# mklarqvist/StormBitmaps

Measured on AMD Instinct MI355X. Metric: 64-bit bitmap words/s, XX^T upper-tri pairwise AND+popcount (10000x65536), higher is better.
Workload: dtype u64 (bits as exact FP4 0/1 MFMA operands, f32 accumulate < 2^24); 1 GPU; STORM_contiguous_t N=10000 M=65536 dense draws=32768 seed=42 (BASELINE configs[1], README `benchmark 65536 10000`); entry_point=storm_hip_pairw_dense_launch == STORM_contig_pairw_intersect_cardinality_blocked, kernel_variant=4, work_items=14520

## Files before the change

### stormbitmaps_amd/csrc/storm_hip_mfma.hip

```cpp
#include "storm_hip_internal.h"

#include <algorithm>
#include <chrono>
#include <cstring>
#include <exception>
#include <type_traits>
#include <utility>

namespace storm {

#ifdef STORM_HIP_PROBES
__device__ unsigned long long g_clock_probe[4];
#define STORM_CLOCK_BEGIN()                                  \
    const uint64_t ck_t0 = __builtin_amdgcn_s_memtime();     \
    const uint64_t ck_r0 = __builtin_amdgcn_s_memrealtime()
#define STORM_CLOCK_END()                                                                           \
    do {                                                                                            \
        if (threadIdx.x == 0) {                                                                     \
            atomicAdd(&g_clock_probe[0], (unsigned long long)(__builtin_amdgcn_s_memtime() - ck_t0)); \
            atomicAdd(&g_clock_probe[1], (unsigned long long)(__builtin_amdgcn_s_memrealtime() - ck_r0)); \
            atomicAdd(&g_clock_probe[2], 1ull);                                                     \
        }                                                                                           \
    } while (0)
#else
#define STORM_CLOCK_BEGIN() do {} while (0)
#define STORM_CLOCK_END() do {} while (0)
#endif

static hipError_t wait_stream(storm_hip_ctx_t* ctx) {
    if (ctx->sync_poll_us > 0) {
        const auto t0 = std::chrono::steady_clock::now();
        for (uint32_t spin = 0;; ++spin) {
            const hipError_t q = hipStreamQuery(ctx->stream);
            if (q != hipErrorNotReady) return q;
            if ((spin & 15u) == 15u &&
                std::chrono::duration<double, std::micro>(std::chrono::steady_clock::now() - t0).count() > ctx->sync_poll_us)
                break;
        }
    }
    return hipStreamSynchronize(ctx->stream);
}

constexpr int kMfmaThreads = 512;
constexpr int kTileStageBytes = kTile * kStageBytes;
constexpr int kRing = 4;

typedef int v8i __attribute__((ext_vector_type(8)));
typedef int v4i __attribute__((ext_vector_type(4)));
typedef float v16f __attribute__((ext_vector_type(16)));

using gptr_t = const __attribute__((address_space(1))) void*;
using lptr_t = __attribute__((address_space(3))) void*;

#include "tile_window.inc"

__device__ __forceinline__ uint32_t spread8_fp4(uint32_t b, uint32_t nib = 2u) {
    uint32_t x = (b | (b << 12)) & 0x000F000Fu;
    x = (x | (x << 6)) & 0x03030303u;
    x = (x | (x << 3)) & 0x11111111u;
    return x * nib;
}

struct ExpandOwn {
    uint32_t rank, count, unit_shift, modulo_units;
};
constexpr ExpandOwn kExpandAll = {0u, 1u, 7u, 0u};

__global__ __launch_bounds__(256) void expand_fp4_kernel(const uint64_t* __restrict__ X,
                                                         uint64_t stride_words,
                                                         uint64_t n_rows_src, uint64_t n_rows_dst,
                                                         uint4* __restrict__ X4, ExpandOwn own,
                                                         uint32_t nib = 2u, uint64_t out_pitch_u4 = 0,
                                                         uint64_t h_begin = 0, uint64_t h_end = 0,
                                                         uint64_t h_dst0 = 0) {
    if (out_pitch_u4 == 0) out_pitch_u4 = stride_words * 2;
    const uint64_t halves_per_row = stride_words * 2;
    if (h_end == 0) h_end = halves_per_row;
    const uint32_t shift = own.unit_shift;
    const uint64_t units = (h_end - h_begin + (1ull << shift) - 1) >> shift;
// ... 379 lines not shown
        STORM_LGKM(0);
    }
#undef STORM_FETCH16
#undef STORM_MUL16
#undef STORM_LGKM
#undef STORM_LGKM_STR

    uint64_t mine = 0;
#pragma unroll
    for (int m = 0; m < 4; ++m) {
        uint32_t part = 0;
#pragma unroll
        for (int n = 0; n < 4; ++n)
#pragma unroll
            for (int r = 0; r < 4; ++r) part += (uint32_t)acc[m][n][r];
        mine += part;
    }
#pragma unroll
    for (int o = 32; o > 0; o >>= 1) mine += __shfl_down(mine, o, 64);
    if (lane == 0 && mine != 0)
        atomicAdd(&slots[(item_idx * (uint32_t)kStripWaves + wave) & (kSlots - 1)],
                  (unsigned long long)mine);
}

constexpr int kSb16ImgRing = 3;
constexpr int kSb16BitRing = 3;
[[maybe_unused]] constexpr int kSb16BitStage = kStripBRows * 64;
constexpr uint32_t kSb16ImgBytes = kSb16ImgRing * kStripStageBytes;
constexpr uint32_t kSb16Mask = 0x22222222u;

__device__ __forceinline__ v4i sb16_inflate(v4i w, uint32_t rot) {
    v4i e;
    e.x = (int)(__builtin_amdgcn_alignbit((uint32_t)w.x, (uint32_t)w.x, rot) & kSb16Mask);
    e.y = (int)(__builtin_amdgcn_alignbit((uint32_t)w.y, (uint32_t)w.y, rot) & kSb16Mask);
    e.z = (int)(__builtin_amdgcn_alignbit((uint32_t)w.z, (uint32_t)w.z, rot) & kSb16Mask);
    e.w = (int)(__builtin_amdgcn_alignbit((uint32_t)w.w, (uint32_t)w.w, rot) & kSb16Mask);
    return e;
}

#define STORM_SB16_WAVES 4
#define STORM_SB16_NAME strip16_bits_kernel
#include "strip16_bits_kernel.inc"
#undef STORM_SB16_WAVES
#undef STORM_SB16_NAME
#define STORM_SB16_WAVES 8
#define STORM_SB16_NAME strip16_bits2_kernel
#include "strip16_bits_kernel.inc"
#undef STORM_SB16_WAVES
#undef STORM_SB16_NAME

constexpr uint32_t kSr16SliceBytes = 16;
constexpr uint32_t kSr16PerTile = kStripRowsATile / kStripBRows;
constexpr uint32_t kSr16StageBytes = kStripBRows * 64;
constexpr uint32_t kSr16ImgBytes = 3 * kSr16StageBytes;
constexpr uint32_t kSr16BitRing = 3;
constexpr uint32_t kSr16BitStage = 4 * 256;

__device__ __forceinline__ v4i sr16_inflate(uint32_t w) {
    v4i e;
    e.x = (int)(__builtin_amdgcn_alignbit(w, w, 31u) & kSb16Mask);
    e.y = (int)(w & kSb16Mask);
    e.z = (int)(__builtin_amdgcn_alignbit(w, w, 1u) & kSb16Mask);
    e.w = (int)(__builtin_amdgcn_alignbit(w, w, 2u) & kSb16Mask);
    return e;
}
#include "strip16_rows_kernel.inc"

[[maybe_unused]] constexpr int kT16Ring = 4;
constexpr int kT16RowBytes = 128;
[[maybe_unused]] constexpr int kT16StageBytes = kTile * kT16RowBytes;

#ifdef STORM_HIP_PROBES
#include "../../tools/probes/tile16_fp4.hip"
#endif

[[maybe_unused]] constexpr int kTbThreads = 256;
constexpr int kTbRing = 4;
constexpr int kTbRowBytes = 64;
constexpr int kTbImageBytes = kTile * kTbRowBytes;
constexpr int kTbStageBytes = 2 * kTbImageBytes;

template <int C>
__device__ __forceinline__ v4i tb_inflate(v4i w) {
    typedef unsigned v4u __attribute__((ext_vector_type(4)));
    if constexpr (C == 3) return (v4i)(((v4u)w >> 1u) & 0x44444444u);
    else return w & (int)(0x11111111u << C);
}
template <int C>
__device__ __forceinline__ int tb_scale() {
    return C == 0 ? 128 : C == 1 ? 127 : 126;
}

template <int MB>
__device__ __forceinline__ void tb_store_interior(const v16f (&acc)[MB][4], uint8_t* lds_wave,
                                                  uint32_t* __restrict__ out_tile, uint64_t ld,
                                                  uint32_t lane, const uint32_t* __restrict__ row_counts,
                                                  uint32_t i0, uint32_t j0, uint32_t and_weight) {
    uint32_t* w32 = reinterpret_cast<uint32_t*>(lds_wave);
    const uint4* r128 = reinterpret_cast<const uint4*>(lds_wave);
    uint32_t nj[4] = {0u, 0u, 0u, 0u};
    if (row_counts) {
#pragma unroll
        for (int n = 0; n < 4; ++n) nj[n] = row_counts[j0 + (uint32_t)n * 32u + (lane & 31u)];
    }
#pragma unroll
    for (int m = 0; m < MB; ++m) {
#pragma unroll
// ... 1586 lines not shown
            l.n = (uint32_t)items.size();
            if (l.n) {
                if (int rc_up = upload_bytes(ctx, l.d, items.data(), items.size() * sizeof(StripItem))) return rc_up;
                STORM_HIP_TRY(hipStreamSynchronize(ctx->stream));
            }
            l.key = rq;
        }
        STORM_HIP_TRY(hipStreamWaitEvent(ctx->stream, l.landed, 0));
        if (l.n) {
            hipLaunchKernelGGL(strip16_bits_kernel, dim3(l.n), dim3(kStripThreads), (size_t)ctx->k2_lds_pad, ctx->stream,
                               reinterpret_cast<const uint8_t*>(m->d), pitch, l.d.d, ctx->d_slots,
                               (unsigned long long*)nullptr, (uint32_t)kSlots);
            STORM_HIP_TRY(hipGetLastError());
        }
        n_total += l.n;
    }
    ctx->last_info[0] = n_total;
    ctx->last_info[1] = ctx->k2_stages_per_item;
    ctx->last_info[2] = 1;
    ctx->last_info[3] = n_panels;
    return launch_fold_slots(ctx, d_total);
}

int strip_operands_of(const storm_hip_ctx_t* ctx) {
    if (ctx->k2_strip_operands == 6) return 5;
    if (ctx->k2_strip_operands != 0) return ctx->k2_strip_operands;
    return (ctx->k2_ring == kStripRingDefault && ctx->k2_shape == 16) ? 5 : 4;
}
int launch_pairw_mfma(storm_hip_ctx_t* ctx, const storm_hip_matrix_s* m, uint32_t shard_rank,
                      uint32_t shard_count, uint64_t* d_total) {
    const int strip_mode = ctx->variant == 5 ? 2 : ctx->variant == 4 ? 1 : 0;
    const int operands = strip_operands_of(ctx);
    if (strip_mode == 1 && (operands == 1 || operands == 2 || operands == 3 || operands == 5) && !ctx->k2_persistent && ctx->k2_debug == 0 &&
        (m->n_rows + kStripATile - 1) / kStripATile * kStripATile <= m->n_rows_pad &&
        m->stride_words * 8 * (uint64_t)kStripBRows < (1ull << 32))
    {
        const bool wide = operands == 5 && ctx->k2_strip_operands == 6 && (m->n_rows + 511u) / 512u * 512u <= m->n_rows_pad;
        ctx->k2_operands_used = wide ? 6 : operands;
        return launch_pairw_bits(ctx, m, shard_rank, shard_count, wide ? 6 : operands, d_total);
    }
    ctx->k2_operands_used = 4;
    const uint64_t tile = strip_mode == 2 ? 512 : kStripATile;
    const uint64_t n_rows4 = (m->n_rows + tile - 1) / tile * tile;
    std::vector<RowRange> ranges;
    if (m->n_rows > 1) ranges.push_back({0, m->n_rows});
    return launch_pairw_mfma_ranges(ctx, m->d, m->stride_words, m->n_rows_pad, n_rows4, ranges,
                                    shard_rank, shard_count, strip_mode, d_total, m->generation,
                                    m->n_words);
}

}

#ifdef STORM_HIP_PROBES
extern "C" int storm_hip_probe_clock(uint64_t out[3]) {
    unsigned long long v[4] = {0, 0, 0, 0};
    if (hipDeviceSynchronize() != hipSuccess) return STORM_HIP_EINVAL;
    if (hipMemcpyFromSymbol(v, HIP_SYMBOL(storm::g_clock_probe), sizeof(v)) != hipSuccess) return STORM_HIP_EINVAL;
    out[0] = v[0];
    out[1] = v[1];
    out[2] = v[2];
    const unsigned long long z[4] = {0, 0, 0, 0};
    if (hipMemcpyToSymbol(HIP_SYMBOL(storm::g_clock_probe), z, sizeof(z)) != hipSuccess) return STORM_HIP_EINVAL;
    return STORM_HIP_OK;
}
#endif
```

### stormbitmaps_amd/csrc/strip16_rows_kernel.inc

```
__global__ __launch_bounds__(256, 4) void strip16_rows_kernel(
    const uint8_t* __restrict__ X, uint64_t row_bytes, const StripItem* __restrict__ items,
    unsigned long long* __restrict__ slots, unsigned long long* __restrict__ out, uint32_t fold_slots) {
    __shared__ __attribute__((aligned(1024))) uint8_t lds_raw[kSr16ImgBytes + kSr16BitRing * kSr16BitStage];

    constexpr uint32_t kW = 4u;
    STORM_CLOCK_BEGIN();
    const uint32_t tid = threadIdx.x;
    const uint32_t lane = tid & 63u;
    const uint32_t wave = __builtin_amdgcn_readfirstlane(tid >> 6);
    const StripItem it = items[blockIdx.x];
    const uint64_t kbyte = (uint64_t)it.ks * (uint64_t)kSr16SliceBytes;
    const uint32_t D = it.diag ? kSr16PerTile : 0u;
    const uint32_t T = D + (it.j1 - it.j0);
    const uint32_t cslot = (3u - D % 3u) % 3u;

    const uint32_t lds_base =
        (uint32_t)(uintptr_t)(__attribute__((address_space(3))) uint8_t*)&lds_raw[0];
    const uint32_t pr = wave * 16u + (lane >> 2);
    const uint32_t goff0 = pr * (uint32_t)row_bytes + (lane & 3u) * 4u;
    const uint32_t bits_rd = lds_base + kSr16ImgBytes + wave * 256u + lane * 4u;
    const uint32_t img_wr = lds_base + pr * 64u + (((lane & 3u) ^ ((0x78u >> (2u * ((pr >> 2) & 3u))) & 3u)) * 16u);

    auto issue = [&](uint32_t s, uint32_t slot) {
        const uint32_t sc = min(s, T - 1u);
        const uint32_t blk = sc < D ? it.a_row0 / (uint32_t)kStripBRows + sc : it.j1 - 1u - (sc - D);
        const uint8_t* base = X + (uint64_t)(blk * (uint32_t)kStripBRows) * row_bytes + kbyte;
        const __amdgpu_buffer_rsrc_t rsrc =
            __builtin_amdgcn_make_buffer_rsrc(const_cast<uint8_t*>(base), 0, -1, 0x00020000);
        __builtin_amdgcn_raw_ptr_buffer_load_lds(
            rsrc, (lptr_t)(lds_raw + kSr16ImgBytes + slot * kSr16BitStage + wave * 256u), 4,
            (int)goff0, 0, 0, 0);
    };

    v4i a[8];
    {
        const uint8_t* ap = X + (uint64_t)(it.a_row0 + wave * 64u + (lane & 15u)) * row_bytes + kbyte +
                            (lane >> 4) * 4u;
        uint32_t aw[8];
#pragma unroll
        for (int m = 0; m < 8; ++m)
            aw[m] = *reinterpret_cast<const uint32_t*>(ap + (uint64_t)((m & 3) * 16 + (m >> 2) * 256) * row_bytes);
        issue(0u, cslot);
        issue(1u, (cslot + 1u) % 3u);
        issue(2u, (cslot + 2u) % 3u);
#pragma unroll
        for (int m = 0; m < 8; ++m) a[m] = sr16_inflate(aw[m]);
    }

    v4f acc[8][2];
#pragma unroll
    for (int m = 0; m < 8; ++m)
#pragma unroll
        for (int n = 0; n < 2; ++n) acc[m][n] = v4f{};

    const uint32_t boff = lds_base + (lane & 15u) * 64u + (((lane >> 4) ^ ((0x78u >> (2u * ((lane & 15u) >> 2))) & 3u)) * 16u);

#pragma unroll
    for (int m = 0; m < 8; ++m) asm volatile("" ::"v"(a[m]));

#define STORM_FETCH16(dst, img, j)                                                        \
    asm volatile("ds_read_b128 %0, %1 offset:%2"                                          \
                 : "=&v"(dst)                                                             \
                 : "v"(boff), "n"((img) + (j) * 16 * 64))
#define STORM_FETCH16V(dst, img, j)                                                       \
    asm volatile("ds_read_b128 %0, %1 offset:%2"                                          \
                 : "=&v"(dst)                                                             \
                 : "v"(boff + (img)), "n"((j) * 16 * 64))
#define STORM_MUL1(m, j, frag)                                                            \
    acc[m][(j) & 1] = __builtin_amdgcn_mfma_scale_f32_16x16x128_f8f6f4(                   \
        v8i{a[m].x, a[m].y, a[m].z, a[m].w, 0, 0, 0, 0},                                  \
        v8i{frag.x, frag.y, frag.z, frag.w, 0, 0, 0, 0}, acc[m][(j) & 1], 4, 4, 0, 0, 0, 0)
#define STORM_MUL16(j, frag)                                                              \
    _Pragma("unroll") for (int m = 0; m < 8; ++m) STORM_MUL1(m, j, frag)
#define STORM_LGKM_STR(n) asm volatile("s_waitcnt lgkmcnt(" #n ")" ::: "memory")
#define STORM_LGKM(n)    \
    STORM_LGKM_STR(n);   \
    __builtin_amdgcn_sched_barrier(0)
#define STORM_VM2()                                         \
    asm volatile("s_waitcnt vmcnt(2)" ::: "memory");        \
    __builtin_amdgcn_sched_barrier(0)

    uint32_t wb = 0;
    auto build_image = [&](uint32_t s) {
        uint32_t slot = (s + cslot) % 3u;
        asm volatile("" : "+s"(slot));
        asm volatile("ds_read_b32 %0, %1" : "=&v"(wb) : "v"(bits_rd + slot * kSr16BitStage));
        STORM_LGKM(0);
        const v4i e = sr16_inflate(wb);
        asm volatile("ds_write_b128 %0, %1" ::"v"(img_wr + slot * kSr16StageBytes), "v"(e) : "memory");
        __builtin_amdgcn_sched_barrier(0);
    };

    asm volatile("s_waitcnt lgkmcnt(0)" ::: "memory");
    STORM_VM2();
    build_image(0u);
    STORM_LGKM(0);
    issue(3u, cslot);
    STORM_VM2();
    build_image(1u);

    v4i b0 = {}, b1 = {}, b2 = {};
    uint32_t t = 0;
    if (D != 0u) {
#define STORM_SR16_MASK(m, n)                                                             \
    _Pragma("unroll") for (int r = 0; r < 4; ++r) acc[m][n][r] = r < tri ? acc[m][n][r] : 0.0f;
#define STORM_SR16_WHOLE(base, j)                                                         \
    _Pragma("unroll") for (int i = 0; i < 4; ++i) {                                       \
        STORM_MUL1((base) + i, j, b0);                                                    \
        STORM_MUL1((base) + i, (j) + 1, b1);                                              \
    }
#define STORM_SR16_OWN01(base)                                                            \
    STORM_MUL1((base) + 0, 0, b0);                                                        \
    STORM_SR16_MASK((base) + 0, 0)                                                        \
    STORM_MUL1((base) + 0, 1, b1);                                                        \
    STORM_MUL1((base) + 1, 1, b1);                                                        \
    STORM_SR16_MASK((base) + 1, 1)
#define STORM_SR16_OWN23(base)                                                            \
    STORM_MUL1((base) + 0, 2, b0);                                                        \
    STORM_MUL1((base) + 1, 2, b0);                                                        \
    STORM_MUL1((base) + 2, 2, b0);                                                        \
    STORM_SR16_MASK((base) + 2, 0)                                                        \
    STORM_MUL1((base) + 0, 3, b1);                                                        \
    STORM_MUL1((base) + 1, 3, b1);                                                        \
    STORM_MUL1((base) + 2, 3, b1);                                                        \
    STORM_MUL1((base) + 3, 3, b1);                                                        \
    STORM_SR16_MASK((base) + 3, 1)
#define STORM_SR16_HEAD()                                                                 \
    STORM_LGKM(0);                                                  \
    __builtin_amdgcn_s_barrier();     \
    issue(t + 4u, (t + 1u + cslot) % 3u);                                                 \
    STORM_VM2();                                                         \
    build_image(t + 2u);                                                                  \
    uint32_t sb = ((t + cslot) % 3u) * kSr16StageBytes;                                   \
    asm volatile("" : "+s"(sb))
#define STORM_SR16_PAIR(j)                                                                \
    __builtin_amdgcn_sched_barrier(0);                                                    \
    STORM_FETCH16V(b0, sb, j);                                                            \
    STORM_FETCH16V(b1, sb, (j) + 1);                                                      \
    STORM_LGKM(0)
#pragma unroll 1
        for (; t < wave; ++t) {
            STORM_SR16_HEAD();
        }
        {
            STORM_SR16_HEAD();
            const uint32_t lane_d = __builtin_amdgcn_mbcnt_hi(~0u, __builtin_amdgcn_mbcnt_lo(~0u, 0u));
            const int tri = (int)(lane_d & 15u) - (int)(4u * (lane_d >> 4));
            STORM_SR16_PAIR(0);
            STORM_SR16_OWN01(0)
            STORM_SR16_PAIR(2);
            STORM_SR16_OWN23(0)
            ++t;
        }
#pragma unroll 1
        for (; t < wave + 4u; ++t) {
            STORM_SR16_HEAD();
            STORM_SR16_PAIR(0);
            STORM_SR16_WHOLE(0, 0)
            STORM_SR16_PAIR(2);
            STORM_SR16_WHOLE(0, 2)
        }
        {
            STORM_SR16_HEAD();
            const uint32_t lane_d = __builtin_amdgcn_mbcnt_hi(~0u, __builtin_amdgcn_mbcnt_lo(~0u, 0u));
            const int tri = (int)(lane_d & 15u) - (int)(4u * (lane_d >> 4));
            STORM_SR16_PAIR(0);
            STORM_SR16_WHOLE(0, 0)
            STORM_SR16_OWN01(4)
            STORM_SR16_PAIR(2);
            STORM_SR16_WHOLE(0, 2)
            STORM_SR16_OWN23(4)
            ++t;
        }
#pragma unroll 1
        for (; t < kSr16PerTile; ++t) {
            STORM_SR16_HEAD();
            STORM_SR16_PAIR(0);
            STORM_SR16_WHOLE(0, 0)
            STORM_SR16_WHOLE(4, 0)
            STORM_SR16_PAIR(2);
            STORM_SR16_WHOLE(0, 2)
            STORM_SR16_WHOLE(4, 2)
        }
        __builtin_amdgcn_sched_barrier(0);
#undef STORM_SR16_PAIR
#undef STORM_SR16_HEAD
#undef STORM_SR16_OWN23
#undef STORM_SR16_OWN01
#undef STORM_SR16_WHOLE
#undef STORM_SR16_MASK
    }
#define STORM_SR16_BODY(I, fa, fb, fc)                                                                      \
    {                                                                                                       \
        issue(t + 4u, ((I) + 1) % 3);              \
        STORM_VM2();                                               \
        asm volatile("ds_read_b32 %0, %1 offset:%2" : "=&v"(wb) : "v"(bits_rd), "n"((((I) + 2) % 3) * kSr16BitStage)); \
        v4i e;                                                                                              \
        STORM_FETCH16(fc, (I) * kSr16StageBytes, 2); STORM_LGKM(3); STORM_MUL16(0, fa); __builtin_amdgcn_sched_barrier(0); \
        STORM_FETCH16(fa, (I) * kSr16StageBytes, 3); STORM_LGKM(2);       \
        e = sr16_inflate(wb); STORM_MUL16(1, fb); __builtin_amdgcn_sched_barrier(0);                        \
        asm volatile("ds_write_b128 %0, %1 offset:%2" ::"v"(img_wr), "v"(e), "n"((((I) + 2) % 3) * kSr16StageBytes) : "memory"); \
        STORM_FETCH16(fb, (((I) + 1) % 3) * kSr16StageBytes, 0); STORM_LGKM(3); STORM_MUL16(2, fc); __builtin_amdgcn_sched_barrier(0); \
        STORM_FETCH16(fc, (((I) + 1) % 3) * kSr16StageBytes, 1); STORM_LGKM(2); STORM_MUL16(3, fa); __builtin_amdgcn_sched_barrier(0); \
        ++t;                                                                                                \
        if (t >= T) break;                                                                                  \
        __builtin_amdgcn_s_barrier();                                                                       \
    }
    if (t < T) {
        STORM_LGKM(0);
        __builtin_amdgcn_s_barrier();
        STORM_FETCH16(b0, 0, 0);
        STORM_FETCH16(b1, 0, 1);
        for (;;) {
            STORM_SR16_BODY(0, b0, b1, b2)
            STORM_SR16_BODY(1, b1, b2, b0)
            STORM_SR16_BODY(2, b2, b0, b1)
        }
        STORM_LGKM(0);
    }
    asm volatile("s_waitcnt vmcnt(0)" ::: "memory");
    asm volatile("" ::"v"(b0), "v"(b1), "v"(b2), "v"(wb));
#undef STORM_SR16_BODY
#undef STORM_VM2
#undef STORM_FETCH16V
#undef STORM_FETCH16
#undef STORM_MUL16
#undef STORM_MUL1
#undef STORM_LGKM
#undef STORM_LGKM_STR

    STORM_CLOCK_END();
    uint64_t mine = 0;
#pragma unroll
    for (int m = 0; m < 8; ++m) {
        uint32_t part = 0;
#pragma unroll
        for (int n = 0; n < 2; ++n)
#pragma unroll
            for (int r = 0; r < 4; ++r) part += (uint32_t)acc[m][n][r];
        mine += part;
    }
#pragma unroll
    for (int o = 32; o > 0; o >>= 1) mine += __shfl_down(mine, o, 64);
    const uint32_t lane_e = __builtin_amdgcn_mbcnt_hi(~0u, __builtin_amdgcn_mbcnt_lo(~0u, 0u));
    const uint32_t tid_e = wave * 64u + lane_e;
    if (out == nullptr) {
        if (lane_e == 0 && mine != 0)
            atomicAdd(&slots[(blockIdx.x * kW + wave) & (kSlots - 1)],
                      (unsigned long long)mine);
        return;
    }
    if (lane_e == 0)
        atomicAdd(&slots[(blockIdx.x * kW + wave) & (fold_slots - 1u)],
                  (unsigned long long)mine + (1ull << 48));
    if (blockIdx.x != gridDim.x - 1u) return;
    const unsigned long long expected = (unsigned long long)gridDim.x * (unsigned long long)kW;
    unsigned long long* wsum = reinterpret_cast<unsigned long long*>(lds_raw);
    unsigned long long total = 0;
    for (;;) {
        unsigned long long cnt = 0, sum = 0;
        for (uint32_t i = tid_e; i < fold_slots; i += (kW * 64u)) {
            const unsigned long long v = __hip_atomic_load(&slots[i], __ATOMIC_RELAXED, __HIP_MEMORY_SCOPE_AGENT);
            cnt += v >> 48;
            sum += v & ((1ull << 48) - 1ull);
        }
#pragma unroll
        for (int o = 32; o > 0; o >>= 1) {
            cnt += __shfl_down(cnt, o, 64);
            sum += __shfl_down(sum, o, 64);
        }
        __syncthreads();
        if (lane_e == 0) {
            wsum[wave] = cnt;
            wsum[kW + wave] = sum;
        }
        __syncthreads();
        cnt = 0;
        total = 0;
#pragma unroll
        for (uint32_t w = 0; w < kW; ++w) {
            cnt += wsum[w];
            total += wsum[kW + w];
        }
        if (cnt == expected) break;
        if (fold_slots > (kW * 64u)) __builtin_amdgcn_s_sleep(8);
    }
    for (uint32_t i = tid_e; i < fold_slots; i += (kW * 64u))
        __hip_atomic_store(&slots[i], 0ull, __ATOMIC_RELAXED, __HIP_MEMORY_SCOPE_AGENT);
    if (tid_e == 0) out[0] = total;
}
```

### stormbitmaps_amd/csrc/storm_hip_plan.h

```cpp
#pragma once

#include <cstdint>
#include <cstring>
#include <type_traits>
#include <utility>
#include <vector>

namespace storm {

void set_error(const char* fmt, ...);
bool timing_env();

template <class T>
inline bool same_request(const T& a, const T& b) {
    static_assert(std::has_unique_object_representations_v<T>, "a request struct with padding cannot be compared with memcmp");
    return !memcmp(&a, &b, sizeof(T));
}

constexpr int kChunkWords = 64;

constexpr int kTile = 256;
constexpr int kStageBytes = 64;
constexpr uint32_t kGroupStages = 32;

struct MfmaItem {
    uint16_t I, J;
    uint32_t stage0;
    uint32_t n_stages;
};
static_assert(sizeof(MfmaItem) == 12, "read by device code");

constexpr uint32_t kOwnSlices = 4;
constexpr int kStripRowBytes = 128;
constexpr int kStripBRows = 64;
constexpr int kStripWaves = 4;
constexpr int kStripATile = 64 * kStripWaves;
constexpr uint32_t kStripRowsATile = 512;
constexpr uint32_t kStripRowsXcdGroup = 8;
inline uint32_t strip_rows_kslices(uint32_t n_words) { return (n_words + 1u) / 2u; }

struct StripItem {
    uint32_t a_row0;
    uint32_t diag;
    uint32_t j0, j1;
    uint32_t ks;
};
static_assert(sizeof(StripItem) == 20, "read by device code");

struct BitSeg {
    uint32_t a_blk;
    uint32_t ks;
    uint32_t b_first;
    uint32_t n_b;
    uint32_t range_b0;
    uint32_t range_nb;
    uint32_t flags;
    uint32_t pad;
};
static_assert(sizeof(BitSeg) == 32, "read by device code");
constexpr uint32_t kBsDiag = 1u;
constexpr uint32_t kBsMaxStages = 8192;

constexpr uint32_t kThTile = 128u;
struct PartItem {
    uint16_t I, J;
    uint32_t stage0, n_stages;
    uint32_t tile;
    uint32_t win0;
    uint16_t part, n_parts;
};
static_assert(sizeof(PartItem) == 24, "read by device code");
constexpr uint16_t kThNarrow = 0x8000u;
constexpr uint32_t kThWeightBits = 512u;
constexpr uint32_t kThWeightDosage = 9u * 256u;

struct RowRange {
    uint64_t r0, r1;
    uint64_t a_end = 0;
    uint64_t back_from = ~0ull;
};
uint64_t ranges_hash(const std::vector<RowRange>& ranges);

inline uint32_t strip_modulo_slices(uint32_t n_kslices, uint32_t shard_count) {
    return n_kslices / kOwnSlices / shard_count * shard_count * kOwnSlices;
}
inline bool strip_owns_slice(uint32_t ks, uint32_t shard_rank, uint32_t shard_count) {
    return (ks / kOwnSlices) % shard_count == shard_rank;
}

struct TileSumRequest {
    uint64_t ranges_hash;
    uint32_t total_stages, shard_rank, shard_count;
// ... 207 lines not shown
```

Measured before the change: 142300 billion words/s.

## Restructure diagonal-tile phase with row-interleaved A layout and symmetric half-sum correction

```diff
diff --git a/stormbitmaps_amd/csrc/storm_hip_mfma.hip b/stormbitmaps_amd/csrc/storm_hip_mfma.hip
--- a/stormbitmaps_amd/csrc/storm_hip_mfma.hip
+++ b/stormbitmaps_amd/csrc/storm_hip_mfma.hip
@@ -22,9 +22,29 @@
             atomicAdd(&g_clock_probe[2], 1ull);                                                     \
         }                                                                                           \
     } while (0)
+__device__ unsigned long long g_phase_probe[4];
+#define STORM_PHASE_BEGIN(var) uint64_t var = ck_r0
+#define STORM_PHASE_STAMP(var)                                  \
+    do {                                                        \
+        var = __builtin_amdgcn_s_memrealtime();                 \
+        asm volatile("s_waitcnt lgkmcnt(0)" : "+s"(var)::"memory"); \
+    } while (0)
+#define STORM_PHASE_END(var, has_diag)                                                              \
+    do {                                                                                            \
+        const uint64_t ph_end = __builtin_amdgcn_s_memrealtime();                                   \
+        if (threadIdx.x == 0) {                                                                     \
+            if (has_diag) atomicAdd(&g_phase_probe[0], (unsigned long long)(var - ck_r0));          \
+            atomicAdd(&g_phase_probe[1], (unsigned long long)(ph_end - ck_r0));                     \
+            if (has_diag) atomicAdd(&g_phase_probe[2], 1ull);                                       \
+            atomicAdd(&g_phase_probe[3], 1ull);                                                     \
+        }                                                                                           \
+    } while (0)
 #else
 #define STORM_CLOCK_BEGIN() do {} while (0)
 #define STORM_CLOCK_END() do {} while (0)
+#define STORM_PHASE_BEGIN(var) do {} while (0)
+#define STORM_PHASE_STAMP(var) do {} while (0)
+#define STORM_PHASE_END(var, has_diag) do {} while (0)
 #endif
 
 static hipError_t wait_stream(storm_hip_ctx_t* ctx) {
@@ -2203,7 +2223,7 @@
 }
 
 #ifdef STORM_HIP_PROBES
-extern "C" int storm_hip_probe_clock(uint64_t out[3]) {
+extern "C" __attribute__((visibility("default"))) int storm_hip_probe_clock(uint64_t out[3]) {
     unsigned long long v[4] = {0, 0, 0, 0};
     if (hipDeviceSynchronize() != hipSuccess) return STORM_HIP_EINVAL;
     if (hipMemcpyFromSymbol(v, HIP_SYMBOL(storm::g_clock_probe), sizeof(v)) != hipSuccess) return STORM_HIP_EINVAL;
@@ -2214,4 +2234,13 @@
     if (hipMemcpyToSymbol(HIP_SYMBOL(storm::g_clock_probe), z, sizeof(z)) != hipSuccess) return STORM_HIP_EINVAL;
     return STORM_HIP_OK;
 }
+extern "C" __attribute__((visibility("default"))) int storm_hip_probe_phase(uint64_t out[4]) {
+    unsigned long long v[4] = {0, 0, 0, 0};
+    if (hipDeviceSynchronize() != hipSuccess) return STORM_HIP_EINVAL;
+    if (hipMemcpyFromSymbol(v, HIP_SYMBOL(storm::g_phase_probe), sizeof(v)) != hipSuccess) return STORM_HIP_EINVAL;
+    for (int i = 0; i < 4; ++i) out[i] = v[i];
+    const unsigned long long z[4] = {0, 0, 0, 0};
+    if (hipMemcpyToSymbol(HIP_SYMBOL(storm::g_phase_probe), z, sizeof(z)) != hipSuccess) return STORM_HIP_EINVAL;
+    return STORM_HIP_OK;
+}
 #endif
diff --git a/stormbitmaps_amd/csrc/strip16_rows_kernel.inc b/stormbitmaps_amd/csrc/strip16_rows_kernel.inc
--- a/stormbitmaps_amd/csrc/strip16_rows_kernel.inc
+++ b/stormbitmaps_amd/csrc/strip16_rows_kernel.inc
@@ -33,25 +33,23 @@
     };
 
     v4i a[8];
+    uint32_t own_pop = 0;
     {
-        const uint8_t* ap = X + (uint64_t)(it.a_row0 + wave * 64u + (lane & 15u)) * row_bytes + kbyte +
+        const uint8_t* ap = X + (uint64_t)(it.a_row0 + wave * 16u + (lane & 15u)) * row_bytes + kbyte +
                             (lane >> 4) * 4u;
         uint32_t aw[8];
 #pragma unroll
         for (int m = 0; m < 8; ++m)
-            aw[m] = *reinterpret_cast<const uint32_t*>(ap + (uint64_t)((m & 3) * 16 + (m >> 2) * 256) * row_bytes);
+            aw[m] = *reinterpret_cast<const uint32_t*>(ap + (uint64_t)(m * 64) * row_bytes);
         issue(0u, cslot);
         issue(1u, (cslot + 1u) % 3u);
         issue(2u, (cslot + 2u) % 3u);
 #pragma unroll
-        for (int m = 0; m < 8; ++m) a[m] = sr16_inflate(aw[m]);
-    }
-
-    v4f acc[8][2];
-#pragma unroll
-    for (int m = 0; m < 8; ++m)
-#pragma unroll
-        for (int n = 0; n < 2; ++n) acc[m][n] = v4f{};
+        for (int m = 0; m < 8; ++m) {
+            a[m] = sr16_inflate(aw[m]);
+            own_pop += (uint32_t)__builtin_popcount(aw[m]);
+        }
+    }
 
     const uint32_t boff = lds_base + (lane & 15u) * 64u + (((lane >> 4) ^ ((0x78u >> (2u * ((lane & 15u) >> 2))) & 3u)) * 16u);
 
@@ -62,10 +60,6 @@
     asm volatile("ds_read_b128 %0, %1 offset:%2"                                          \
                  : "=&v"(dst)                                                             \
                  : "v"(boff), "n"((img) + (j) * 16 * 64))
-#define STORM_FETCH16V(dst, img, j)                                                       \
-    asm volatile("ds_read_b128 %0, %1 offset:%2"                                          \
-                 : "=&v"(dst)                                                             \
-                 : "v"(boff + (img)), "n"((j) * 16 * 64))
 #define STORM_MUL1(m, j, frag)                                                            \
     acc[m][(j) & 1] = __builtin_amdgcn_mfma_scale_f32_16x16x128_f8f6f4(                   \
         v8i{a[m].x, a[m].y, a[m].z, a[m].w, 0, 0, 0, 0},                                  \
@@ -99,96 +93,100 @@
     STORM_VM2();
     build_image(1u);
 
+    v4f acc[8][2];
+#pragma unroll
+    for (int m = 0; m < 8; ++m)
+#pragma unroll
+        for (int n = 0; n < 2; ++n) acc[m][n] = v4f{};
+
     v4i b0 = {}, b1 = {}, b2 = {};
     uint32_t t = 0;
+    STORM_PHASE_BEGIN(ph_diag);
+    int32_t own_x = 0;
     if (D != 0u) {
-#define STORM_SR16_MASK(m, n)                                                             \
-    _Pragma("unroll") for (int r = 0; r < 4; ++r) acc[m][n][r] = r < tri ? acc[m][n][r] : 0.0f;
-#define STORM_SR16_WHOLE(base, j)                                                         \
-    _Pragma("unroll") for (int i = 0; i < 4; ++i) {                                       \
-        STORM_MUL1((base) + i, j, b0);                                                    \
-        STORM_MUL1((base) + i, (j) + 1, b1);                                              \
-    }
-#define STORM_SR16_OWN01(base)                                                            \
-    STORM_MUL1((base) + 0, 0, b0);                                                        \
-    STORM_SR16_MASK((base) + 0, 0)                                                        \
-    STORM_MUL1((base) + 0, 1, b1);                                                        \
-    STORM_MUL1((base) + 1, 1, b1);                                                        \
-    STORM_SR16_MASK((base) + 1, 1)
-#define STORM_SR16_OWN23(base)                                                            \
-    STORM_MUL1((base) + 0, 2, b0);                                                        \
-    STORM_MUL1((base) + 1, 2, b0);                                                        \
-    STORM_MUL1((base) + 2, 2, b0);                                                        \
-    STORM_SR16_MASK((base) + 2, 0)                                                        \
-    STORM_MUL1((base) + 0, 3, b1);                                                        \
-    STORM_MUL1((base) + 1, 3, b1);                                                        \
-    STORM_MUL1((base) + 2, 3, b1);                                                        \
-    STORM_MUL1((base) + 3, 3, b1);                                                        \
-    STORM_SR16_MASK((base) + 3, 1)
-#define STORM_SR16_HEAD()                                                                 \
-    STORM_LGKM(0);                                                  \
-    __builtin_amdgcn_s_barrier();     \
-    issue(t + 4u, (t + 1u + cslot) % 3u);                                                 \
-    STORM_VM2();                                                         \
-    build_image(t + 2u);                                                                  \
-    uint32_t sb = ((t + cslot) % 3u) * kSr16StageBytes;                                   \
-    asm volatile("" : "+s"(sb))
-#define STORM_SR16_PAIR(j)                                                                \
-    __builtin_amdgcn_sched_barrier(0);                                                    \
-    STORM_FETCH16V(b0, sb, j);                                                            \
-    STORM_FETCH16V(b1, sb, (j) + 1);                                                      \
-    STORM_LGKM(0)
-#pragma unroll 1
-        for (; t < wave; ++t) {
-            STORM_SR16_HEAD();
-        }
+        acc[7][1][0] = -(float)own_pop;
+        uint32_t so0 = wave * 1024u, so1 = ((wave + 1u) & 3u) * 1024u, so2 = ((wave + 2u) & 3u) * 1024u;
+#define STORM_FETCH16O(dst, img, so)                                                      \
+    asm volatile("" : "+s"(so));    \
+    asm volatile("ds_read_b128 %0, %1 offset:%2" : "=&v"(dst) : "v"(boff + (so)), "n"(img))
+#define STORM_SR16_WHOLE(d, j, frag)                                                      \
+    _Pragma("unroll") for (int m = 0; m < (d); ++m) STORM_MUL1(m, j, frag)
+#define STORM_SR16_OWNH(d, frag)                                                          \
+    acc[7][1] = __builtin_amdgcn_mfma_scale_f32_16x16x128_f8f6f4(                         \
+        v8i{a[d].x, a[d].y, a[d].z, a[d].w, 0, 0, 0, 0},                                  \
+        v8i{frag.x, frag.y, frag.z, frag.w, 0, 0, 0, 0}, acc[7][1], 4, 4, 0, 0, 0, 0)
+#define STORM_SR16_DIAG(d, I, fa, fb, fc)                                                                   \
+    {                                                                                                       \
+        issue((d) + 4u, ((I) + 1) % 3);                                                                     \
+        STORM_VM2();                                               \
+        asm volatile("ds_read_b32 %0, %1 offset:%2" : "=&v"(wb) : "v"(bits_rd), "n"((((I) + 2) % 3) * kSr16BitStage)); \
+        STORM_LGKM(2); STORM_SR16_WHOLE(d, 0, fa); __builtin_amdgcn_sched_barrier(0);                       \
+        STORM_LGKM(0);                                                        \
+        {                                                                                                   \
+            const v4i e = sr16_inflate(wb);                                                                 \
+            asm volatile("ds_write_b128 %0, %1 offset:%2" ::"v"(img_wr), "v"(e), "n"((((I) + 2) % 3) * kSr16StageBytes) : "memory"); \
+        }                                                                                                   \
+        __builtin_amdgcn_sched_barrier(0);                                                                  \
+        STORM_FETCH16(fa, (I) * kSr16StageBytes, 2);                                                        \
+        STORM_FETCH16(fc, (I) * kSr16StageBytes, 3);                                                        \
+        STORM_SR16_WHOLE(d, 1, fb); __builtin_amdgcn_sched_barrier(0);                                      \
+        STORM_FETCH16O(fb, (I) * kSr16StageBytes, so0); STORM_LGKM(2); STORM_SR16_WHOLE(d, 2, fa); __builtin_amdgcn_sched_barrier(0); \
+        STORM_FETCH16O(fa, (I) * kSr16StageBytes, so1); STORM_LGKM(2); STORM_SR16_WHOLE(d, 3, fc); __builtin_amdgcn_sched_barrier(0); \
+        STORM_FETCH16O(fc, (I) * kSr16StageBytes, so2); STORM_LGKM(2); STORM_SR16_OWNH(d, fb); __builtin_amdgcn_sched_barrier(0); \
+        STORM_FETCH16(fb, (((I) + 1) % 3) * kSr16StageBytes, 0); STORM_LGKM(2); STORM_MUL1(d, 0, fa); __builtin_amdgcn_sched_barrier(0); \
+        STORM_FETCH16(fa, (((I) + 1) % 3) * kSr16StageBytes, 1); STORM_LGKM(2); STORM_SR16_OWNH(d, fc); __builtin_amdgcn_sched_barrier(0); \
+        __builtin_amdgcn_s_barrier();                                                                       \
+    }
+        STORM_LGKM(0);
+        __builtin_amdgcn_s_barrier();
+        STORM_FETCH16O(b0, 1 * kSr16StageBytes, so0);
+        STORM_FETCH16O(b1, 1 * kSr16StageBytes, so1);
         {
-            STORM_SR16_HEAD();
-            const uint32_t lane_d = __builtin_amdgcn_mbcnt_hi(~0u, __builtin_amdgcn_mbcnt_lo(~0u, 0u));
-            const int tri = (int)(lane_d & 15u) - (int)(4u * (lane_d >> 4));
-            STORM_SR16_PAIR(0);
-            STORM_SR16_OWN01(0)
-            STORM_SR16_PAIR(2);
-            STORM_SR16_OWN23(0)
-            ++t;
-        }
-#pragma unroll 1
-        for (; t < wave + 4u; ++t) {
-            STORM_SR16_HEAD();
-            STORM_SR16_PAIR(0);
-            STORM_SR16_WHOLE(0, 0)
-            STORM_SR16_PAIR(2);
-            STORM_SR16_WHOLE(0, 2)
-        }
-        {
-            STORM_SR16_HEAD();
-            const uint32_t lane_d = __builtin_amdgcn_mbcnt_hi(~0u, __builtin_amdgcn_mbcnt_lo(~0u, 0u));
-            const int tri = (int)(lane_d & 15u) - (int)(4u * (lane_d >> 4));
-            STORM_SR16_PAIR(0);
-            STORM_SR16_WHOLE(0, 0)
-            STORM_SR16_OWN01(4)
-            STORM_SR16_PAIR(2);
-            STORM_SR16_WHOLE(0, 2)
-            STORM_SR16_OWN23(4)
-            ++t;
-        }
-#pragma unroll 1
-        for (; t < kSr16PerTile; ++t) {
-            STORM_SR16_HEAD();
-            STORM_SR16_PAIR(0);
-            STORM_SR16_WHOLE(0, 0)
-            STORM_SR16_WHOLE(4, 0)
-            STORM_SR16_PAIR(2);
-            STORM_SR16_WHOLE(0, 2)
-            STORM_SR16_WHOLE(4, 2)
-        }
+            issue(4u, 2u);
+            STORM_VM2();
+            asm volatile("ds_read_b32 %0, %1 offset:%2" : "=&v"(wb) : "v"(bits_rd), "n"(0 * kSr16BitStage));
+            STORM_LGKM(2); STORM_SR16_OWNH(0, b0); __builtin_amdgcn_sched_barrier(0);
+            STORM_LGKM(0);
+            {
+                const v4i e = sr16_inflate(wb);
+                asm volatile("ds_write_b128 %0, %1 offset:%2" ::"v"(img_wr), "v"(e), "n"(0 * kSr16StageBytes) : "memory");
+            }
+            __builtin_amdgcn_sched_barrier(0);
+            STORM_FETCH16O(b0, 1 * kSr16StageBytes, so2);
+            STORM_MUL1(0, 0, b1); __builtin_amdgcn_sched_barrier(0);
+            STORM_FETCH16(b1, 2 * kSr16StageBytes, 0); STORM_LGKM(1); STORM_SR16_OWNH(0, b0); __builtin_amdgcn_sched_barrier(0);
+            STORM_FETCH16(b0, 2 * kSr16StageBytes, 1);
+            __builtin_amdgcn_s_barrier();
+        }
+        STORM_SR16_DIAG(1, 2, b1, b0, b2)
+        STORM_SR16_DIAG(2, 0, b0, b1, b2)
+        STORM_SR16_DIAG(3, 1, b1, b0, b2)
+        STORM_SR16_DIAG(4, 2, b0, b1, b2)
+        STORM_SR16_DIAG(5, 0, b1, b0, b2)
+        STORM_SR16_DIAG(6, 1, b0, b1, b2)
+        int32_t xl = 0;
+#pragma unroll
+        for (int r = 0; r < 4; ++r) xl += (int32_t)acc[7][1][r];
+        acc[7][1] = v4f{};
+        STORM_SR16_DIAG(7, 2, b1, b0, b2)
+        t = kSr16PerTile;
         __builtin_amdgcn_sched_barrier(0);
-#undef STORM_SR16_PAIR
-#undef STORM_SR16_HEAD
-#undef STORM_SR16_OWN23
-#undef STORM_SR16_OWN01
+#undef STORM_SR16_DIAG
+#undef STORM_SR16_OWNH
 #undef STORM_SR16_WHOLE
-#undef STORM_SR16_MASK
+#undef STORM_FETCH16O
+        STORM_PHASE_STAMP(ph_diag);
+#pragma unroll
+        for (int r = 0; r < 4; ++r) xl += (int32_t)acc[7][1][r];
+        acc[7][1] = v4f{};
+#pragma unroll
+        for (int o = 32; o > 0; o >>= 1) xl += __shfl_down(xl, o, 64);
+        own_x = __builtin_amdgcn_readfirstlane(xl);
+    } else if (T != 0u) {
+        STORM_LGKM(0);
+        __builtin_amdgcn_s_barrier();
+        STORM_FETCH16(b0, 0, 0);
+        STORM_FETCH16(b1, 0, 1);
     }
 #define STORM_SR16_BODY(I, fa, fb, fc)                                                                      \
     {                                                                                                       \
@@ -206,29 +204,29 @@
         if (t >= T) break;                                                                                  \
         __builtin_amdgcn_s_barrier();                                                                       \
     }
+#pragma unroll
+    for (int m = 0; m < 8; ++m)
+#pragma unroll
+        for (int n = 0; n < 2; ++n) asm volatile("" : "+v"(acc[m][n]));
     if (t < T) {
-        STORM_LGKM(0);
-        __builtin_amdgcn_s_barrier();
-        STORM_FETCH16(b0, 0, 0);
-        STORM_FETCH16(b1, 0, 1);
         for (;;) {
             STORM_SR16_BODY(0, b0, b1, b2)
             STORM_SR16_BODY(1, b1, b2, b0)
             STORM_SR16_BODY(2, b2, b0, b1)
         }
-        STORM_LGKM(0);
-    }
+    }
+    STORM_LGKM(0);
     asm volatile("s_waitcnt vmcnt(0)" ::: "memory");
     asm volatile("" ::"v"(b0), "v"(b1), "v"(b2), "v"(wb));
 #undef STORM_SR16_BODY
 #undef STORM_VM2
-#undef STORM_FETCH16V
 #undef STORM_FETCH16
 #undef STORM_MUL16
 #undef STORM_MUL1
 #undef STORM_LGKM
 #undef STORM_LGKM_STR
 
+    STORM_PHASE_END(ph_diag, D != 0u);
     STORM_CLOCK_END();
     uint64_t mine = 0;
 #pragma unroll
@@ -242,6 +240,7 @@
     }
 #pragma unroll
     for (int o = 32; o > 0; o >>= 1) mine += __shfl_down(mine, o, 64);
+    mine += (uint64_t)((uint32_t)own_x + (wave < 2u ? 1u : 0u)) >> 1;
     const uint32_t lane_e = __builtin_amdgcn_mbcnt_hi(~0u, __builtin_amdgcn_mbcnt_lo(~0u, 0u));
     const uint32_t tid_e = wave * 64u + lane_e;
     if (out == nullptr) {
```

After: 143200 billion words/s (median of 6 runs). No clear change (+0.7%).

## Build diagonal tile from resident A fragments in LDS instead of streaming B

Applied to the files above, without the earlier changes.

```diff
diff --git a/stormbitmaps_amd/csrc/storm_hip_mfma.hip b/stormbitmaps_amd/csrc/storm_hip_mfma.hip
--- a/stormbitmaps_amd/csrc/storm_hip_mfma.hip
+++ b/stormbitmaps_amd/csrc/storm_hip_mfma.hip
@@ -510,7 +510,7 @@
 constexpr uint32_t kSr16SliceBytes = 16;
 constexpr uint32_t kSr16PerTile = kStripRowsATile / kStripBRows;
 constexpr uint32_t kSr16StageBytes = kStripBRows * 64;
-constexpr uint32_t kSr16ImgBytes = 3 * kSr16StageBytes;
+constexpr uint32_t kSr16ImgBytes = kSr16PerTile * kSr16StageBytes;
 constexpr uint32_t kSr16BitRing = 3;
 constexpr uint32_t kSr16BitStage = 4 * 256;
 
diff --git a/stormbitmaps_amd/csrc/storm_hip_plan.h b/stormbitmaps_amd/csrc/storm_hip_plan.h
--- a/stormbitmaps_amd/csrc/storm_hip_plan.h
+++ b/stormbitmaps_amd/csrc/storm_hip_plan.h
@@ -38,6 +38,21 @@
 constexpr uint32_t kStripRowsATile = 512;
 constexpr uint32_t kStripRowsXcdGroup = 8;
 inline uint32_t strip_rows_kslices(uint32_t n_words) { return (n_words + 1u) / 2u; }
+constexpr uint32_t kStripRowsBlocks = kStripRowsATile / (uint32_t)kStripBRows;
+constexpr uint32_t kStripRowsWaves = 4;
+enum StripRowsRole : uint32_t { kStripRowsSkip = 0, kStripRowsOwn = 1, kStripRowsWhole = 2 };
+constexpr uint32_t strip_rows_block(uint32_t wave, uint32_t half) { return half ? kStripRowsBlocks - 1u - wave : wave; }
+constexpr StripRowsRole strip_rows_role(uint32_t wave, uint32_t half, uint32_t d) {
+    return d < strip_rows_block(wave, half) ? kStripRowsSkip : d == strip_rows_block(wave, half) ? kStripRowsOwn : kStripRowsWhole;
+}
+constexpr uint32_t strip_rows_diag_begin(uint32_t wave) {
+    return strip_rows_block(wave, 0) < strip_rows_block(wave, 1) ? strip_rows_block(wave, 0) : strip_rows_block(wave, 1);
+}
+constexpr uint32_t strip_rows_diag_end(uint32_t) { return kStripRowsBlocks; }
+constexpr uint32_t strip_rows_role_mfmas(StripRowsRole r) { return r == kStripRowsWhole ? 16u : r == kStripRowsOwn ? 10u : 0u; }
+static_assert(strip_rows_block(0, 0) < strip_rows_block(0, 1) && strip_rows_block(1, 0) < strip_rows_block(1, 1) &&
+              strip_rows_block(2, 0) < strip_rows_block(2, 1) && strip_rows_block(3, 0) < strip_rows_block(3, 1),
+              "strip16_rows_kernel walks the low half's own block first");
 
 struct StripItem {
     uint32_t a_row0;
diff --git a/stormbitmaps_amd/csrc/strip16_rows_kernel.inc b/stormbitmaps_amd/csrc/strip16_rows_kernel.inc
--- a/stormbitmaps_amd/csrc/strip16_rows_kernel.inc
+++ b/stormbitmaps_amd/csrc/strip16_rows_kernel.inc
@@ -3,16 +3,18 @@
     unsigned long long* __restrict__ slots, unsigned long long* __restrict__ out, uint32_t fold_slots) {
     __shared__ __attribute__((aligned(1024))) uint8_t lds_raw[kSr16ImgBytes + kSr16BitRing * kSr16BitStage];
 
-    constexpr uint32_t kW = 4u;
+    constexpr uint32_t kW = kStripRowsWaves;
+    static_assert(kSr16PerTile == kStripRowsBlocks && kSr16ImgBytes >= kStripRowsBlocks * kSr16StageBytes, "eight resident images");
     STORM_CLOCK_BEGIN();
     const uint32_t tid = threadIdx.x;
     const uint32_t lane = tid & 63u;
     const uint32_t wave = __builtin_amdgcn_readfirstlane(tid >> 6);
     const StripItem it = items[blockIdx.x];
     const uint64_t kbyte = (uint64_t)it.ks * (uint64_t)kSr16SliceBytes;
-    const uint32_t D = it.diag ? kSr16PerTile : 0u;
-    const uint32_t T = D + (it.j1 - it.j0);
-    const uint32_t cslot = (3u - D % 3u) % 3u;
+    const uint32_t T = it.j1 - it.j0;
+    const uint32_t s_last = T ? T - 1u : 0u;
+    const uint32_t blk_top = T ? it.j1 - 1u : it.a_row0 / (uint32_t)kStripBRows;
+    const uint32_t blk_lo = strip_rows_block(wave, 0u), blk_hi = strip_rows_block(wave, 1u);
 
     const uint32_t lds_base =
         (uint32_t)(uintptr_t)(__attribute__((address_space(3))) uint8_t*)&lds_raw[0];
@@ -22,8 +24,7 @@
     const uint32_t img_wr = lds_base + pr * 64u + (((lane & 3u) ^ ((0x78u >> (2u * ((pr >> 2) & 3u))) & 3u)) * 16u);
 
     auto issue = [&](uint32_t s, uint32_t slot) {
-        const uint32_t sc = min(s, T - 1u);
-        const uint32_t blk = sc < D ? it.a_row0 / (uint32_t)kStripBRows + sc : it.j1 - 1u - (sc - D);
+        const uint32_t blk = blk_top - min(s, s_last);
         const uint8_t* base = X + (uint64_t)(blk * (uint32_t)kStripBRows) * row_bytes + kbyte;
         const __amdgpu_buffer_rsrc_t rsrc =
             __builtin_amdgcn_make_buffer_rsrc(const_cast<uint8_t*>(base), 0, -1, 0x00020000);
@@ -34,15 +35,15 @@
 
     v4i a[8];
     {
-        const uint8_t* ap = X + (uint64_t)(it.a_row0 + wave * 64u + (lane & 15u)) * row_bytes + kbyte +
-                            (lane >> 4) * 4u;
+        const uint8_t* ap = X + (uint64_t)(it.a_row0 + (lane & 15u)) * row_bytes + kbyte + (lane >> 4) * 4u;
         uint32_t aw[8];
 #pragma unroll
         for (int m = 0; m < 8; ++m)
-            aw[m] = *reinterpret_cast<const uint32_t*>(ap + (uint64_t)((m & 3) * 16 + (m >> 2) * 256) * row_bytes);
-        issue(0u, cslot);
-        issue(1u, (cslot + 1u) % 3u);
-        issue(2u, (cslot + 2u) % 3u);
+            aw[m] = *reinterpret_cast<const uint32_t*>(
+                ap + (uint64_t)((m < 4 ? blk_lo : blk_hi) * (uint32_t)kStripBRows + (uint32_t)(m & 3) * 16u) * row_bytes);
+        issue(0u, 0u);
+        issue(1u, 1u);
+        issue(2u, 2u);
 #pragma unroll
         for (int m = 0; m < 8; ++m) a[m] = sr16_inflate(aw[m]);
     }
@@ -82,7 +83,7 @@
 
     uint32_t wb = 0;
     auto build_image = [&](uint32_t s) {
-        uint32_t slot = (s + cslot) % 3u;
+        uint32_t slot = s % 3u;
         asm volatile("" : "+s"(slot));
         asm volatile("ds_read_b32 %0, %1" : "=&v"(wb) : "v"(bits_rd + slot * kSr16BitStage));
         STORM_LGKM(0);
@@ -92,98 +93,75 @@
     };
 
     asm volatile("s_waitcnt lgkmcnt(0)" ::: "memory");
-    STORM_VM2();
-    build_image(0u);
-    STORM_LGKM(0);
-    issue(3u, cslot);
-    STORM_VM2();
-    build_image(1u);
-
-    v4i b0 = {}, b1 = {}, b2 = {};
+
+    v4i b0 = {}, b1 = {}, b2 = {}, b3 = {};
     uint32_t t = 0;
-    if (D != 0u) {
+    if (it.diag) {
+#pragma unroll
+        for (int m = 0; m < 8; ++m) {
+            uint32_t ib = (m < 4 ? blk_lo : blk_hi) * kSr16StageBytes;
+            asm volatile("" : "+s"(ib));
+            asm volatile("ds_write_b128 %0, %1 offset:%2" ::"v"(boff + ib), "v"(a[m]), "n"((m & 3) * 16 * 64) : "memory");
+        }
+        STORM_LGKM(0);
+        __builtin_amdgcn_s_barrier();
 #define STORM_SR16_MASK(m, n)                                                             \
     _Pragma("unroll") for (int r = 0; r < 4; ++r) acc[m][n][r] = r < tri ? acc[m][n][r] : 0.0f;
-#define STORM_SR16_WHOLE(base, j)                                                         \
-    _Pragma("unroll") for (int i = 0; i < 4; ++i) {                                       \
-        STORM_MUL1((base) + i, j, b0);                                                    \
-        STORM_MUL1((base) + i, (j) + 1, b1);                                              \
-    }
-#define STORM_SR16_OWN01(base)                                                            \
-    STORM_MUL1((base) + 0, 0, b0);                                                        \
-    STORM_SR16_MASK((base) + 0, 0)                                                        \
-    STORM_MUL1((base) + 0, 1, b1);                                                        \
-    STORM_MUL1((base) + 1, 1, b1);                                                        \
-    STORM_SR16_MASK((base) + 1, 1)
-#define STORM_SR16_OWN23(base)                                                            \
-    STORM_MUL1((base) + 0, 2, b0);                                                        \
-    STORM_MUL1((base) + 1, 2, b0);                                                        \
-    STORM_MUL1((base) + 2, 2, b0);                                                        \
-    STORM_SR16_MASK((base) + 2, 0)                                                        \
-    STORM_MUL1((base) + 0, 3, b1);                                                        \
-    STORM_MUL1((base) + 1, 3, b1);                                                        \
-    STORM_MUL1((base) + 2, 3, b1);                                                        \
-    STORM_MUL1((base) + 3, 3, b1);                                                        \
-    STORM_SR16_MASK((base) + 3, 1)
+#define STORM_SR16_WHOLE(base, j, frag)                                                   \
+    _Pragma("unroll") for (int i = 0; i < 4; ++i) STORM_MUL1((base) + i, j, frag);
+#define STORM_SR16_OWN01(base, j, frag)                                                   \
+    _Pragma("unroll") for (int i = 0; i <= (j); ++i) STORM_MUL1((base) + i, j, frag);     \
+    STORM_SR16_MASK((base) + (j), j)
+#define STORM_SR16_OWN23(base, j, frag)                                                   \
+    _Pragma("unroll") for (int i = 0; i <= (j); ++i) STORM_MUL1((base) + i, j, frag);     \
+    STORM_SR16_MASK((base) + (j), (j) - 2)
 #define STORM_SR16_HEAD()                                                                 \
-    STORM_LGKM(0);                                                  \
-    __builtin_amdgcn_s_barrier();     \
-    issue(t + 4u, (t + 1u + cslot) % 3u);                                                 \
-    STORM_VM2();                                                         \
-    build_image(t + 2u);                                                                  \
-    uint32_t sb = ((t + cslot) % 3u) * kSr16StageBytes;                                   \
-    asm volatile("" : "+s"(sb))
-#define STORM_SR16_PAIR(j)                                                                \
+    uint32_t sb = d * kSr16StageBytes;                                                    \
+    asm volatile("" : "+s"(sb));                                                          \
     __builtin_amdgcn_sched_barrier(0);                                                    \
-    STORM_FETCH16V(b0, sb, j);                                                            \
-    STORM_FETCH16V(b1, sb, (j) + 1);                                                      \
-    STORM_LGKM(0)
-#pragma unroll 1
-        for (; t < wave; ++t) {
-            STORM_SR16_HEAD();
-        }
+    STORM_FETCH16V(b0, sb, 0);                                                            \
+    STORM_FETCH16V(b1, sb, 1);                                                            \
+    STORM_FETCH16V(b2, sb, 2);                                                            \
+    STORM_FETCH16V(b3, sb, 3)
+        uint32_t d = strip_rows_diag_begin(wave);
         {
             STORM_SR16_HEAD();
             const uint32_t lane_d = __builtin_amdgcn_mbcnt_hi(~0u, __builtin_amdgcn_mbcnt_lo(~0u, 0u));
             const int tri = (int)(lane_d & 15u) - (int)(4u * (lane_d >> 4));
-            STORM_SR16_PAIR(0);
-            STORM_SR16_OWN01(0)
-            STORM_SR16_PAIR(2);
-            STORM_SR16_OWN23(0)
-            ++t;
+            STORM_LGKM(3); STORM_SR16_OWN01(0, 0, b0) __builtin_amdgcn_sched_barrier(0);
+            STORM_LGKM(2); STORM_SR16_OWN01(0, 1, b1) __builtin_amdgcn_sched_barrier(0);
+            STORM_LGKM(1); STORM_SR16_OWN23(0, 2, b2) __builtin_amdgcn_sched_barrier(0);
+            STORM_LGKM(0); STORM_SR16_OWN23(0, 3, b3) __builtin_amdgcn_sched_barrier(0);
+            ++d;
         }
 #pragma unroll 1
-        for (; t < wave + 4u; ++t) {
-            STORM_SR16_HEAD();
-            STORM_SR16_PAIR(0);
-            STORM_SR16_WHOLE(0, 0)
-            STORM_SR16_PAIR(2);
-            STORM_SR16_WHOLE(0, 2)
+        for (; d < blk_hi; ++d) {
+            STORM_SR16_HEAD();
+            STORM_LGKM(3); STORM_SR16_WHOLE(0, 0, b0) __builtin_amdgcn_sched_barrier(0);
+            STORM_LGKM(2); STORM_SR16_WHOLE(0, 1, b1) __builtin_amdgcn_sched_barrier(0);
+            STORM_LGKM(1); STORM_SR16_WHOLE(0, 2, b2) __builtin_amdgcn_sched_barrier(0);
+            STORM_LGKM(0); STORM_SR16_WHOLE(0, 3, b3) __builtin_amdgcn_sched_barrier(0);
         }
         {
             STORM_SR16_HEAD();
             const uint32_t lane_d = __builtin_amdgcn_mbcnt_hi(~0u, __builtin_amdgcn_mbcnt_lo(~0u, 0u));
             const int tri = (int)(lane_d & 15u) - (int)(4u * (lane_d >> 4));
-            STORM_SR16_PAIR(0);
-            STORM_SR16_WHOLE(0, 0)
-            STORM_SR16_OWN01(4)
-            STORM_SR16_PAIR(2);
-            STORM_SR16_WHOLE(0, 2)
-            STORM_SR16_OWN23(4)
-            ++t;
+            STORM_LGKM(3); STORM_SR16_WHOLE(0, 0, b0) STORM_SR16_OWN01(4, 0, b0) __builtin_amdgcn_sched_barrier(0);
+            STORM_LGKM(2); STORM_SR16_WHOLE(0, 1, b1) STORM_SR16_OWN01(4, 1, b1) __builtin_amdgcn_sched_barrier(0);
+            STORM_LGKM(1); STORM_SR16_WHOLE(0, 2, b2) STORM_SR16_OWN23(4, 2, b2) __builtin_amdgcn_sched_barrier(0);
+            STORM_LGKM(0); STORM_SR16_WHOLE(0, 3, b3) STORM_SR16_OWN23(4, 3, b3) __builtin_amdgcn_sched_barrier(0);
+            ++d;
         }
 #pragma unroll 1
-        for (; t < kSr16PerTile; ++t) {
-            STORM_SR16_HEAD();
-            STORM_SR16_PAIR(0);
-            STORM_SR16_WHOLE(0, 0)
-            STORM_SR16_WHOLE(4, 0)
-            STORM_SR16_PAIR(2);
-            STORM_SR16_WHOLE(0, 2)
-            STORM_SR16_WHOLE(4, 2)
+        for (; d < strip_rows_diag_end(wave); ++d) {
+            STORM_SR16_HEAD();
+            STORM_LGKM(3); STORM_MUL16(0, b0); __builtin_amdgcn_sched_barrier(0);
+            STORM_LGKM(2); STORM_MUL16(1, b1); __builtin_amdgcn_sched_barrier(0);
+            STORM_LGKM(1); STORM_MUL16(2, b2); __builtin_amdgcn_sched_barrier(0);
+            STORM_LGKM(0); STORM_MUL16(3, b3); __builtin_amdgcn_sched_barrier(0);
         }
         __builtin_amdgcn_sched_barrier(0);
-#undef STORM_SR16_PAIR
+        __builtin_amdgcn_s_barrier();
 #undef STORM_SR16_HEAD
 #undef STORM_SR16_OWN23
 #undef STORM_SR16_OWN01
@@ -206,7 +184,13 @@
         if (t >= T) break;                                                                                  \
         __builtin_amdgcn_s_barrier();                                                                       \
     }
-    if (t < T) {
+    if (T != 0u) {
+        STORM_VM2();
+        build_image(0u);
+        STORM_LGKM(0);
+        issue(3u, 0u);
+        STORM_VM2();
+        build_image(1u);
         STORM_LGKM(0);
         __builtin_amdgcn_s_barrier();
         STORM_FETCH16(b0, 0, 0);
@@ -219,7 +203,7 @@
         STORM_LGKM(0);
     }
     asm volatile("s_waitcnt vmcnt(0)" ::: "memory");
-    asm volatile("" ::"v"(b0), "v"(b1), "v"(b2), "v"(wb));
+    asm volatile("" ::"v"(b0), "v"(b1), "v"(b2), "v"(b3), "v"(wb));
 #undef STORM_SR16_BODY
 #undef STORM_VM2
 #undef STORM_FETCH16V
```

After: 141400 billion words/s before, 144500 billion words/s after, median of 6. 1.02x the previous value.
